# sangminwoo/Temporal-Span-Proposal-Network-VidVRD

Measured on AMD Instinct MI355X. Metric: tracklet-pairs/sec scored (N=32, T=150, D=2048), higher is better.
Workload: dtype f32

## Files before the change

temporal-span-proposal-network-vidvrd_amd/csrc/tspn_linear.hip:

```cpp
#include <algorithm>

#include "tspn_common.h"
#include "tspn_span_pool.h"
#include "tspn_device.h"

namespace {

using namespace tspn_dev;

constexpr int TM = 64;
constexpr int NBLK = 9;
constexpr int TN = 16 * NBLK;
constexpr int KC = 32;
constexpr int LDS_STRIDE = KC + 2;
constexpr int THREADS = 256;
constexpr int MAX_SPLIT = 64;

constexpr int MAX_NORM_SPLITS = 128;
struct SplitTable {
  int n;
  int kbeg[MAX_NORM_SPLITS];
  int kend[MAX_NORM_SPLITS];
  short blk[MAX_NORM_SPLITS];
};

template <bool NORM>
__global__ __launch_bounds__(THREADS) void linear_splitk_kernel(
    const float* __restrict__ x, int64_t P, int64_t F, int64_t ldx, const float* __restrict__ W,
    int64_t ldw, int64_t K, int64_t k_per_split, float* __restrict__ partial, SplitTable tab,
    float* __restrict__ norm_partial) {
  __shared__ float xs[TM * LDS_STRIDE];
  __shared__ float wsm[TN * LDS_STRIDE];

  const int tid = threadIdx.x;
  const int lane = tid & 63, wave = tid >> 6;
  const int li = lane & 15, kq = lane >> 4;
  const int64_t row0 = (int64_t)blockIdx.x * TM;
  const int64_t col0 = (int64_t)blockIdx.y * TN;
  int64_t kbeg, kend;
  if (NORM) {
    kbeg = tab.kbeg[blockIdx.z];
    kend = tab.kend[blockIdx.z];
  } else {
    kbeg = (int64_t)blockIdx.z * k_per_split;
    kend = (kbeg + k_per_split < F) ? kbeg + k_per_split : F;
  }
  float asum[TM / 8];
#pragma unroll
  for (int r = 0; r < TM / 8; ++r) asum[r] = 0.f;

  f32x4 acc[NBLK];
#pragma unroll
  for (int nb = 0; nb < NBLK; ++nb)
#pragma unroll
    for (int e = 0; e < 4; ++e) acc[nb][e] = 0.f;

  const int lk = tid & 31;
  const int lr = tid >> 5;

  for (int64_t k0 = kbeg; k0 < kend; k0 += KC) {
    const int64_t k = k0 + lk;
    const bool kv = k < kend;
#pragma unroll
    for (int r = 0; r < TM / 8; ++r) {
      const int row = lr + 8 * r;
      const int64_t gr = row0 + row;
      const float xv = (kv && gr < P) ? x[gr * ldx + k] : 0.f;
      xs[row * LDS_STRIDE + lk] = xv;
      if (NORM) asum[r] += fabsf(xv);
    }
#pragma unroll
    for (int r = 0; r < TN / 8; ++r) {
      const int row = lr + 8 * r;
      const int64_t gc = col0 + row;
      wsm[row * LDS_STRIDE + lk] = (kv && gc < K) ? W[gc * ldw + k] : 0.f;
    }
    __syncthreads();
#pragma unroll
    for (int kk = 0; kk < KC / 4; ++kk) {
      const float av = xs[(wave * 16 + li) * LDS_STRIDE + kk * 4 + kq];
#pragma unroll
      for (int nb = 0; nb < NBLK; ++nb) {
        const float bv = wsm[(nb * 16 + li) * LDS_STRIDE + kk * 4 + kq];
        acc[nb] = __builtin_amdgcn_mfma_f32_16x16x4f32(av, bv, acc[nb], 0, 0, 0);
      }
    }
    __syncthreads();
  }

  if (NORM && blockIdx.y == 0) {
#pragma unroll
    for (int r = 0; r < TM / 8; ++r) {
      float a = asum[r];
#pragma unroll
      for (int off = 16; off > 0; off >>= 1) a += __shfl_xor(a, off);
      const int64_t gr = row0 + lr + 8 * r;
      if (lk == 0 && gr < P) norm_partial[(int64_t)blockIdx.z * P + gr] = a;
    }
  }
  float* dst = partial + (int64_t)blockIdx.z * P * K;
#pragma unroll
  for (int nb = 0; nb < NBLK; ++nb) {
    const int64_t gc = col0 + nb * 16 + li;
    if (gc >= K) continue;
#pragma unroll
    for (int e = 0; e < 4; ++e) {
      const int64_t gr = row0 + wave * 16 + kq * 4 + e;
      if (gr < P) dst[gr * K + gc] = acc[nb][e];
    }
  }
}

__global__ void linear_reduce_kernel(const float* __restrict__ partial, int64_t PK, int64_t K,
                                     int splits, const float* __restrict__ b, int apply_sigmoid,
                                     float* __restrict__ out) {
  for (int64_t i = blockIdx.x * (int64_t)blockDim.x + threadIdx.x; i < PK;
       i += (int64_t)gridDim.x * blockDim.x) {
    float s = 0.f;
    for (int z = 0; z < splits; ++z) s += partial[(int64_t)z * PK + i];
    if (b != nullptr) s += b[i % K];
    if (apply_sigmoid) s = 1.f / (1.f + expf(-s));
    out[i] = s;
  }
}

__global__ void linear_reduce_norm_kernel(const float* __restrict__ partial,
                                          const float* __restrict__ norm_partial, int64_t P,
                                          int64_t K, SplitTable tab, const float* __restrict__ b,
                                          int apply_sigmoid, float* __restrict__ out) {
  const int64_t PK = P * K;
  for (int64_t i = blockIdx.x * (int64_t)blockDim.x + threadIdx.x; i < PK;
       i += (int64_t)gridDim.x * blockDim.x) {
    const int64_t row = i / K;
    float s = 0.f;
    int z = 0;
    while (z < tab.n) {
      const int blk = tab.blk[z];
      float acc = 0.f, l1 = 0.f;
      int z2 = z;
      for (; z2 < tab.n && tab.blk[z2] == blk; ++z2) {
        acc += partial[(int64_t)z2 * PK + i];
        if (blk >= 0) l1 += norm_partial[(int64_t)z2 * P + row];
      }
      if (blk >= 0) acc = acc / (l1 == 0.f ? 1.f : l1);
      s += acc;
      z = z2;
    }
    if (b != nullptr) s += b[i % K];
    if (apply_sigmoid) s = 1.f / (1.f + expf(-s));
    out[i] = s;
  }
}

int build_split_table(int64_t P, int64_t F, int64_t K, int64_t first, int64_t block, int64_t nblocks,
                      SplitTable* tab) {
  const int64_t tiles = tspn::ceil_div(P, TM) * tspn::ceil_div(K, TN);
  int64_t target = std::min<int64_t>(std::max<int64_t>(tspn::ceil_div(512, tiles), 1), 64);
  const int64_t len = std::max<int64_t>(tspn::ceil_div(tspn::ceil_div(F, target), KC) * KC, 2 * KC);
  int n = 0;
  auto add_region = [&](int64_t lo, int64_t hi, int blk) {
    if (hi <= lo) return true;
    const int64_t pieces = tspn::ceil_div(hi - lo, len);
    const int64_t step = tspn::ceil_div(tspn::ceil_div(hi - lo, pieces), KC) * KC;
    for (int64_t k = lo; k < hi; k += step) {
      if (n >= MAX_NORM_SPLITS) return false;
      tab->kbeg[n] = (int)k;
      tab->kend[n] = (int)std::min<int64_t>(k + step, hi);
      tab->blk[n] = (short)blk;
      ++n;
    }
    return true;
  };
  bool ok = add_region(0, first, -1);
  for (int64_t bl = 0; ok && bl < nblocks; ++bl)
    ok = add_region(first + bl * block, first + (bl + 1) * block, (int)bl);
  ok = ok && add_region(first + nblocks * block, F, -1);
  tab->n = n;
  return ok ? n : -1;
}

__global__ void pair_combine_kernel(const float* __restrict__ rs, const float* __restrict__ ro,
                                    const int64_t* __restrict__ pairs, int64_t P, int64_t K,
                                    const float* __restrict__ b, float* __restrict__ out) {
  const int64_t total = P * K;
  for (int64_t i = blockIdx.x * (int64_t)blockDim.x + threadIdx.x; i < total;
       i += (int64_t)gridDim.x * blockDim.x) {
    const int64_t p = i / K, k = i - p * K;
    float v = rs[pairs[2 * p] * K + k] + ro[pairs[2 * p + 1] * K + k];
    if (b != nullptr) v += b[k];
    out[i] = 1.f / (1.f + expf(-v));
  }
}

__global__ void span_prefix_kernel(const float* __restrict__ G, int64_t NT, int T, int K2,
                                   double* __restrict__ PS) {
  const int64_t total = NT * K2;
  for (int64_t i = blockIdx.x * (int64_t)blockDim.x + threadIdx.x; i < total;
       i += (int64_t)gridDim.x * blockDim.x) {
    const int64_t trk = i / K2, c = i - trk * K2;
    const float* g = G + (trk * T) * (int64_t)K2 + c;
    double* ps = PS + (trk * (T + 1)) * (int64_t)K2 + c;
    double acc = 0.0;
    ps[0] = 0.0;
    for (int t = 0; t < T; ++t) {
      acc += (double)g[(int64_t)t * K2];
      ps[(int64_t)(t + 1) * K2] = acc;
    }
  }
}

__global__ void span_combine_kernel(const double* __restrict__ PS, const float* __restrict__ G,
                                    const int64_t* __restrict__ pairs, const int64_t* __restrict__ spans,
                                    int64_t P, int T, int K, const float* __restrict__ b,
                                    float* __restrict__ out) {
  const int64_t total = P * K;
  const int64_t K2 = 2 * (int64_t)K;
  for (int64_t i = blockIdx.x * (int64_t)blockDim.x + threadIdx.x; i < total;
       i += (int64_t)gridDim.x * blockDim.x) {
    const int64_t p = i / K, k = i - p * K;
    out[i] = tspn::span_logit(PS, G, pairs[2 * p], pairs[2 * p + 1], spans[2 * p], spans[2 * p + 1], T, K2, k, b);
  }
}

int choose_splits(int64_t P, int64_t F, int64_t K) {
  const int64_t tiles = tspn::ceil_div(P, TM) * tspn::ceil_div(K, TN);
  int64_t s = tspn::ceil_div(512, tiles);
  s = std::min<int64_t>(s, std::max<int64_t>(1, F / (2 * KC)));
  s = std::min<int64_t>(s, MAX_SPLIT);
  return (int)std::max<int64_t>(s, 1);
}

}

extern "C" size_t tspn_predicate_head_workspace_bytes(int64_t P, int64_t F, int64_t K) {
  if (P <= 0 || F <= 0 || K <= 0) return 0;
  return (size_t)choose_splits(P, F, K) * (size_t)P * (size_t)K * sizeof(float);
}

extern "C" int tspn_predicate_head_f32(const float* x, int64_t P, int64_t F, int64_t ldx,
                                       const float* W, const float* b, int64_t K, float* out,
                                       int apply_sigmoid, void* workspace, size_t workspace_bytes,
                                       void* stream) {
  return tspn::linear(x, P, F, ldx, W, F, b, K, out, apply_sigmoid, workspace, workspace_bytes, stream);
}

int tspn::linear(const float* x, int64_t P, int64_t F, int64_t ldx, const float* W, int64_t ldw,
                 const float* b, int64_t K, float* out, int apply_sigmoid, void* workspace,
                 size_t workspace_bytes, void* stream) {
  TSPN_REQUIRE(ldw >= F, TSPN_EINVAL, "tspn_predicate_head_f32: bad ldw");
  TSPN_REQUIRE(P >= 0 && F > 0 && K > 0 && ldx >= F, TSPN_EINVAL,
               "tspn_predicate_head_f32: bad sizes P=%lld F=%lld K=%lld ldx=%lld", (long long)P,
               (long long)F, (long long)K, (long long)ldx);
  if (P == 0) return TSPN_OK;
  TSPN_REQUIRE(x && W && out, TSPN_EINVAL, "tspn_predicate_head_f32: null pointer");
  const int splits = choose_splits(P, F, K);
  const size_t need = (size_t)splits * (size_t)P * (size_t)K * sizeof(float);
  TSPN_REQUIRE(workspace != nullptr && workspace_bytes >= need, TSPN_EWORKSPACE,
               "tspn_predicate_head_f32: workspace %zu < %zu bytes", workspace_bytes, need);
  int64_t kps = tspn::ceil_div(F, splits);
  kps = tspn::ceil_div(kps, KC) * KC;
  const int64_t gx = tspn::ceil_div(P, TM), gy = tspn::ceil_div(K, TN);
  TSPN_REQUIRE(gx < (1LL << 31) && gy < 65536, TSPN_EUNSUPPORTED,
               "tspn_predicate_head_f32: grid too large");
  hipStream_t s = TSPN_STREAM(stream);
  float* partial = static_cast<float*>(workspace);
  hipLaunchKernelGGL(linear_splitk_kernel<false>, dim3((unsigned)gx, (unsigned)gy, (unsigned)splits),
                     dim3(THREADS), 0, s, x, P, F, ldx, W, ldw, K, kps, partial, SplitTable{},
                     (float*)nullptr);
  int rc = tspn::check_launch("tspn_predicate_head_f32(splitk)");
  if (rc) return rc;
  const int64_t PK = P * K;
  const int blocks = (int)std::min<int64_t>(tspn::ceil_div(PK, 256), 4096);
  hipLaunchKernelGGL(linear_reduce_kernel, dim3(blocks), dim3(256), 0, s, partial, PK, K, splits,
                     b, apply_sigmoid, out);
  return tspn::check_launch("tspn_predicate_head_f32(reduce)");
}

extern "C" size_t tspn_predicate_head_norm_workspace_bytes(int64_t P, int64_t F, int64_t K,
                                                           int64_t first, int64_t block,
                                                           int64_t nblocks) {
  if (P <= 0 || F <= 0 || K <= 0 || first < 0 || block <= 0 || nblocks < 0 ||
      first + block * nblocks > F)
    return 0;
  SplitTable tab;
  const int n = build_split_table(P, F, K, first, block, nblocks, &tab);
  if (n < 0) return 0;
  return (size_t)n * (size_t)P * (size_t)(K + 1) * sizeof(float);
}

extern "C" int tspn_predicate_head_norm_f32(const float* x, int64_t P, int64_t F, int64_t ldx,
                                            const float* W, const float* b, int64_t K,
                                            int64_t first, int64_t block, int64_t nblocks,
                                            float* out, int apply_sigmoid, void* workspace,
                                            size_t workspace_bytes, void* stream) {
  TSPN_REQUIRE(P >= 0 && F > 0 && K > 0 && ldx >= F, TSPN_EINVAL,
               "tspn_predicate_head_norm_f32: bad sizes P=%lld F=%lld K=%lld ldx=%lld", (long long)P,
               (long long)F, (long long)K, (long long)ldx);
  TSPN_REQUIRE(first >= 0 && block > 0 && nblocks >= 0 && first + block * nblocks <= F, TSPN_EINVAL,
               "tspn_predicate_head_norm_f32: blocks [%lld, %lld) exceed F=%lld", (long long)first,
               (long long)(first + block * nblocks), (long long)F);
  TSPN_REQUIRE(F < (1LL << 31) && nblocks < 32768, TSPN_EUNSUPPORTED,
               "tspn_predicate_head_norm_f32: F or nblocks too large");
  if (P == 0) return TSPN_OK;
  TSPN_REQUIRE(x && W && out, TSPN_EINVAL, "tspn_predicate_head_norm_f32: null pointer");
  SplitTable tab;
  const int n = build_split_table(P, F, K, first, block, nblocks, &tab);
  TSPN_REQUIRE(n > 0, TSPN_EUNSUPPORTED, "tspn_predicate_head_norm_f32: more than %d K-slices needed",
               MAX_NORM_SPLITS);
  const size_t need = (size_t)n * (size_t)P * (size_t)(K + 1) * sizeof(float);
  TSPN_REQUIRE(workspace != nullptr && workspace_bytes >= need, TSPN_EWORKSPACE,
               "tspn_predicate_head_norm_f32: workspace %zu < %zu bytes", workspace_bytes, need);
  const int64_t gx = tspn::ceil_div(P, TM), gy = tspn::ceil_div(K, TN);
  TSPN_REQUIRE(gx < (1LL << 31) && gy < 65536, TSPN_EUNSUPPORTED,
               "tspn_predicate_head_norm_f32: grid too large");
  hipStream_t s = TSPN_STREAM(stream);
  float* partial = static_cast<float*>(workspace);
  float* norm_partial = partial + (size_t)n * P * K;
  hipLaunchKernelGGL(linear_splitk_kernel<true>, dim3((unsigned)gx, (unsigned)gy, (unsigned)n),
                     dim3(THREADS), 0, s, x, P, F, ldx, W, F, K, (int64_t)0, partial, tab, norm_partial);
  int rc = tspn::check_launch("tspn_predicate_head_norm_f32(splitk)");
  if (rc) return rc;
  const int blocks = (int)std::min<int64_t>(tspn::ceil_div(P * K, 256), 4096);
  hipLaunchKernelGGL(linear_reduce_norm_kernel, dim3(blocks), dim3(256), 0, s, partial, norm_partial,
                     P, K, tab, b, apply_sigmoid, out);
  return tspn::check_launch("tspn_predicate_head_norm_f32(reduce)");
}

size_t tspn::pair_predicate_workspace_bytes(int64_t NT, int64_t D, int64_t K) {
  return tspn::align_up(tspn_predicate_head_workspace_bytes(NT, D, K), 256) +
         2 * tspn::align_up((size_t)NT * K * sizeof(float), 256);
}

int tspn::pair_predicate(const float* fbar, int64_t NT, int64_t D, const int64_t* pairs, int64_t P,
                         const float* cls_w, const float* cls_b, int64_t K, float* out,
                         void* workspace, size_t workspace_bytes, void* stream) {
  if (P == 0 || NT == 0) return TSPN_OK;
  const size_t lin = tspn::align_up(tspn_predicate_head_workspace_bytes(NT, D, K), 256);
  const size_t rbytes = tspn::align_up((size_t)NT * K * sizeof(float), 256);
  TSPN_REQUIRE(workspace && workspace_bytes >= lin + 2 * rbytes, TSPN_EWORKSPACE,
               "pair_predicate: workspace too small");
  char* ws = static_cast<char*>(workspace);
  float* rs = reinterpret_cast<float*>(ws + lin);
  float* ro = reinterpret_cast<float*>(ws + lin + rbytes);
  int rc = tspn::linear(fbar, NT, D, D, cls_w, 2 * D, nullptr, K, rs, 0, ws, lin, stream);
  if (rc) return rc;
  rc = tspn::linear(fbar, NT, D, D, cls_w + D, 2 * D, nullptr, K, ro, 0, ws, lin, stream);
  if (rc) return rc;
  const int blocks = (int)std::min<int64_t>(tspn::ceil_div(P * K, 256), 4096);
  hipLaunchKernelGGL(pair_combine_kernel, dim3(blocks), dim3(256), 0, TSPN_STREAM(stream), rs, ro, pairs,
                     P, K, cls_b, out);
  return tspn::check_launch("pair_predicate(combine)");
}

namespace {
struct SpanLayout {
  size_t lin, g, ps, total;
};
SpanLayout span_layout(int64_t NT, int64_t T, int64_t D, int64_t K) {
  SpanLayout L{};
  L.lin = tspn::align_up(tspn_predicate_head_workspace_bytes(NT * T, D, 2 * K), 256);
  L.g = tspn::align_up((size_t)NT * T * 2 * K * sizeof(float), 256);
  L.ps = tspn::align_up((size_t)NT * (T + 1) * 2 * K * sizeof(double), 256);
  L.total = L.lin + L.g + L.ps;
  return L;
}
}

size_t tspn::span_prefix_workspace_bytes(int64_t NT, int64_t T, int64_t D, int64_t K) {
  if (NT <= 0 || T <= 0 || D <= 0 || K <= 0) return 0;
  return span_layout(NT, T, D, K).total;
}

int tspn::span_prefix_stage(const float* feats, int64_t NT, int64_t T, int64_t D, const float* cls_w, int64_t K,
                            void* workspace, size_t workspace_bytes, void* stream, const float** G_out,
                            const double** PS_out, const char* who) {
  const SpanLayout L = span_layout(NT, T, D, K);
  TSPN_REQUIRE(workspace && workspace_bytes >= L.total, TSPN_EWORKSPACE, "%s: workspace %zu < %zu bytes", who,
               workspace_bytes, L.total);
  char* ws = static_cast<char*>(workspace);
  float* G = reinterpret_cast<float*>(ws + L.lin);
  double* PS = reinterpret_cast<double*>(ws + L.lin + L.g);
  int rc = tspn::linear(feats, NT * T, D, D, cls_w, D, nullptr, 2 * K, G, 0, ws, L.lin, stream);
  if (rc) return rc;
  const int b1 = (int)std::min<int64_t>(tspn::ceil_div(NT * 2 * K, 256), 8192);
  hipLaunchKernelGGL(span_prefix_kernel, dim3(b1), dim3(256), 0, TSPN_STREAM(stream), G, NT, (int)T, (int)(2 * K), PS);
  if ((rc = tspn::check_launch("tspn_span_predicate_f32(prefix)"))) return rc;
  *G_out = G;
  *PS_out = PS;
  return TSPN_OK;
}

extern "C" size_t tspn_span_predicate_workspace_bytes(int64_t NT, int64_t T, int64_t D, int64_t K) {
  return tspn::span_prefix_workspace_bytes(NT, T, D, K);
}

extern "C" int tspn_span_predicate_f32(const float* feats, int64_t NT, int64_t T, int64_t D,
                                       const int64_t* pairs, const int64_t* spans, int64_t P,
                                       const float* cls_w, const float* cls_b, int64_t K, float* out,
                                       void* workspace, size_t workspace_bytes, void* stream) {
  TSPN_REQUIRE(NT >= 0 && T > 0 && D > 0 && K > 0 && P >= 0 && T < (1 << 30) && K < (1 << 20), TSPN_EINVAL,
               "tspn_span_predicate_f32: bad sizes NT=%lld T=%lld D=%lld K=%lld P=%lld", (long long)NT,
               (long long)T, (long long)D, (long long)K, (long long)P);
  if (P == 0 || NT == 0) return TSPN_OK;
  TSPN_REQUIRE(feats && pairs && spans && cls_w && out, TSPN_EINVAL, "tspn_span_predicate_f32: null pointer");
  const float* G = nullptr;
  const double* PS = nullptr;
  int rc = tspn::span_prefix_stage(feats, NT, T, D, cls_w, K, workspace, workspace_bytes, stream, &G, &PS,
                                   "tspn_span_predicate_f32");
  if (rc) return rc;
  hipStream_t s = TSPN_STREAM(stream);
  const int b2 = (int)std::min<int64_t>(tspn::ceil_div(P * K, 256), 8192);
  hipLaunchKernelGGL(span_combine_kernel, dim3(b2), dim3(256), 0, s, PS, G, pairs, spans, P, (int)T,
                     (int)K, cls_b, out);
  return tspn::check_launch("tspn_span_predicate_f32(combine)");
}
```

temporal-span-proposal-network-vidvrd_amd/csrc/tspn_topk_select.h:

```cpp
#pragma once
#include "tspn_common.h"

namespace tspn {

constexpr unsigned kPadKey = 0u;
constexpr int kPadIdx = 0x7fffffff;

template <int THREADS>
__device__ __forceinline__ void bitonic_sort_desc(unsigned* key, int* idx, int n2) {
  const int tid = threadIdx.x;
  for (int k = 2; k <= n2; k <<= 1) {
    for (int j = k >> 1; j > 0; j >>= 1) {
      for (int i = tid; i < n2; i += THREADS) {
        const int l = i ^ j;
        if (l > i) {
          const unsigned ki = key[i], kl = key[l];
          const int ii = idx[i], il = idx[l];
          const bool fwd = (i & k) == 0;
          const bool swap = fwd ? key_before(kl, il, ki, ii) : key_before(ki, ii, kl, il);
          if (swap) {
            key[i] = kl;
            key[l] = ki;
            idx[i] = il;
            idx[l] = ii;
          }
        }
      }
      __syncthreads();
    }
  }
}

constexpr int kRowTopkVPT = 4;
constexpr int kRowTopkMaxK = 64 * kRowTopkVPT;

template <class Emit>
__device__ __forceinline__ void wave_row_topk(const float (&v)[kRowTopkVPT], int K, int R, int lane, Emit emit) {
  unsigned kv[kRowTopkVPT];
#pragma unroll
  for (int i = 0; i < kRowTopkVPT; ++i) kv[i] = order_key(v[i]);
  unsigned used = 0;
  for (int r = 0; r < R; ++r) {
    unsigned bk = kPadKey;
    int bi = kPadIdx;
#pragma unroll
    for (int i = 0; i < kRowTopkVPT; ++i) {
      const int k = lane + 64 * i;
      if (k < K && !((used >> i) & 1u) && key_before(kv[i], k, bk, bi)) {
        bk = kv[i];
        bi = k;
      }
    }
#pragma unroll
    for (int off = 32; off > 0; off >>= 1) {
      const unsigned ok = __shfl_xor(bk, off);
      const int oi = __shfl_xor(bi, off);
      if (key_before(ok, oi, bk, bi)) {
        bk = ok;
        bi = oi;
      }
    }
    if ((bi & 63) == lane && bi < K) {
      float bv = v[0];
#pragma unroll
      for (int i = 1; i < kRowTopkVPT; ++i)
        if ((bi >> 6) == i) bv = v[i];
      used |= 1u << (bi >> 6);
      emit(r, bv, bi);
    }
  }
}

constexpr int kSelectThreads = 1024;
constexpr int kSelectMaxM = 1024;

struct SelectLds {
  unsigned hist[256];
  unsigned prefix, need, count;
  unsigned kk[kSelectMaxM];
  int ki[kSelectMaxM];
};

template <class KeyFn>
__device__ __forceinline__ void select_topk_sorted(SelectLds& L, KeyFn key, int Q, int M) {
  const int tid = threadIdx.x;
  if (tid == 0) {
    L.prefix = 0;
    L.need = (unsigned)M;
  }
  __syncthreads();
  for (int pass = 0; pass < 4; ++pass) {
    const int shift = 24 - 8 * pass;
    if (tid < 256) L.hist[tid] = 0;
    __syncthreads();
    const unsigned prefix = L.prefix;
    const unsigned himask = pass == 0 ? 0u : (0xffffffffu << (shift + 8));
    for (int i = tid; i < Q; i += kSelectThreads) {
      const unsigned k = key(i);
      if ((k & himask) == prefix) atomicAdd(&L.hist[(k >> shift) & 255u], 1u);
    }
    __syncthreads();
    if (tid == 0) {
      unsigned need = L.need, acc = 0;
      int b = 255;
      for (; b >= 0; --b) {
        if (acc + L.hist[b] >= need) break;
        acc += L.hist[b];
      }
      L.prefix = prefix | ((unsigned)b << shift);
      L.need = need - acc;
    }
    __syncthreads();
  }
  const unsigned kth = L.prefix;
  const unsigned ties_needed = L.need;
  __syncthreads();
  if (tid == 0) {
    L.prefix = 0;
    L.need = ties_needed;
  }
  __syncthreads();
  for (int pass = 0; pass < 4; ++pass) {
    const int shift = 24 - 8 * pass;
    if (tid < 256) L.hist[tid] = 0;
    __syncthreads();
    const unsigned prefix = L.prefix;
    const unsigned himask = pass == 0 ? 0u : (0xffffffffu << (shift + 8));
    for (int i = tid; i < Q; i += kSelectThreads) {
      if (key(i) == kth && (((unsigned)i) & himask) == prefix)
        atomicAdd(&L.hist[(((unsigned)i) >> shift) & 255u], 1u);
    }
    __syncthreads();
    if (tid == 0) {
      unsigned need = L.need, acc = 0;
      int b = 0;
      for (; b < 256; ++b) {
        if (acc + L.hist[b] >= need) break;
        acc += L.hist[b];
      }
      L.prefix = prefix | ((unsigned)b << shift);
      L.need = need - acc;
    }
    __syncthreads();
  }
  const unsigned last_tie_idx = L.prefix;

  if (tid == 0) L.count = 0;
  __syncthreads();
  for (int i = tid; i < Q; i += kSelectThreads) {
    const unsigned k = key(i);
    if (k > kth || (k == kth && (unsigned)i <= last_tie_idx)) {
      const unsigned slot = atomicAdd(&L.count, 1u);
      if (slot < (unsigned)kSelectMaxM) {
        L.kk[slot] = k;
        L.ki[slot] = i;
      }
    }
  }
  __syncthreads();
  const int m2 = (int)next_pow2(M);
  for (int i = tid; i < m2; i += kSelectThreads)
    if (i >= M) {
      L.kk[i] = kPadKey;
      L.ki[i] = kPadIdx;
    }
  __syncthreads();
  bitonic_sort_desc<kSelectThreads>(L.kk, L.ki, m2);
}

__device__ inline int argmax_first(const float* p, int n) {
  unsigned bk = order_key(p[0]);
  int bi = 0;
  for (int i = 1; i < n; ++i) {
    const unsigned k = order_key(p[i]);
    if (k > bk) {
      bk = k;
      bi = i;
    }
  }
  return bi;
}

}
```

Baseline: 1.287 million.

## Batch pair-predicate GEMM halves and parallelize top-k selection primitives

```diff
diff --git a/temporal-span-proposal-network-vidvrd_amd/csrc/tspn_linear.hip b/temporal-span-proposal-network-vidvrd_amd/csrc/tspn_linear.hip
--- a/temporal-span-proposal-network-vidvrd_amd/csrc/tspn_linear.hip
+++ b/temporal-span-proposal-network-vidvrd_amd/csrc/tspn_linear.hip
@@ -28,7 +28,7 @@
 __global__ __launch_bounds__(THREADS) void linear_splitk_kernel(
     const float* __restrict__ x, int64_t P, int64_t F, int64_t ldx, const float* __restrict__ W,
     int64_t ldw, int64_t K, int64_t k_per_split, float* __restrict__ partial, SplitTable tab,
-    float* __restrict__ norm_partial) {
+    float* __restrict__ norm_partial, int gy, int64_t w_half, int64_t partial_half) {
   __shared__ float xs[TM * LDS_STRIDE];
   __shared__ float wsm[TN * LDS_STRIDE];
 
@@ -36,7 +36,9 @@
   const int lane = tid & 63, wave = tid >> 6;
   const int li = lane & 15, kq = lane >> 4;
   const int64_t row0 = (int64_t)blockIdx.x * TM;
-  const int64_t col0 = (int64_t)blockIdx.y * TN;
+  const int half = (int)blockIdx.y / gy;
+  const int64_t col0 = (int64_t)((int)blockIdx.y - half * gy) * TN;
+  W += half * w_half;
   int64_t kbeg, kend;
   if (NORM) {
     kbeg = tab.kbeg[blockIdx.z];
@@ -98,7 +100,7 @@
       if (lk == 0 && gr < P) norm_partial[(int64_t)blockIdx.z * P + gr] = a;
     }
   }
-  float* dst = partial + (int64_t)blockIdx.z * P * K;
+  float* dst = partial + half * partial_half + (int64_t)blockIdx.z * P * K;
 #pragma unroll
   for (int nb = 0; nb < NBLK; ++nb) {
     const int64_t gc = col0 + nb * 16 + li;
@@ -113,14 +115,16 @@
 
 __global__ void linear_reduce_kernel(const float* __restrict__ partial, int64_t PK, int64_t K,
                                      int splits, const float* __restrict__ b, int apply_sigmoid,
-                                     float* __restrict__ out) {
-  for (int64_t i = blockIdx.x * (int64_t)blockDim.x + threadIdx.x; i < PK;
-       i += (int64_t)gridDim.x * blockDim.x) {
+                                     float* __restrict__ out, int halves, int64_t partial_half, int64_t out_half) {
+  for (int64_t j = blockIdx.x * (int64_t)blockDim.x + threadIdx.x; j < halves * PK;
+       j += (int64_t)gridDim.x * blockDim.x) {
+    const int64_t half = j / PK, i = j - half * PK;
+    const float* src = partial + half * partial_half;
     float s = 0.f;
-    for (int z = 0; z < splits; ++z) s += partial[(int64_t)z * PK + i];
+    for (int z = 0; z < splits; ++z) s += src[(int64_t)z * PK + i];
     if (b != nullptr) s += b[i % K];
     if (apply_sigmoid) s = 1.f / (1.f + expf(-s));
-    out[i] = s;
+    out[half * out_half + i] = s;
   }
 }
 
@@ -244,9 +248,10 @@
   return tspn::linear(x, P, F, ldx, W, F, b, K, out, apply_sigmoid, workspace, workspace_bytes, stream);
 }
 
-int tspn::linear(const float* x, int64_t P, int64_t F, int64_t ldx, const float* W, int64_t ldw,
-                 const float* b, int64_t K, float* out, int apply_sigmoid, void* workspace,
-                 size_t workspace_bytes, void* stream) {
+namespace {
+int linear_halves(const float* x, int64_t P, int64_t F, int64_t ldx, const float* W, int64_t ldw, const float* b,
+                  int64_t K, float* out, int apply_sigmoid, void* workspace, size_t workspace_bytes, void* stream,
+                  int halves, int64_t w_half, int64_t out_half) {
   TSPN_REQUIRE(ldw >= F, TSPN_EINVAL, "tspn_predicate_head_f32: bad ldw");
   TSPN_REQUIRE(P >= 0 && F > 0 && K > 0 && ldx >= F, TSPN_EINVAL,
                "tspn_predicate_head_f32: bad sizes P=%lld F=%lld K=%lld ldx=%lld", (long long)P,
@@ -254,26 +259,34 @@
   if (P == 0) return TSPN_OK;
   TSPN_REQUIRE(x && W && out, TSPN_EINVAL, "tspn_predicate_head_f32: null pointer");
   const int splits = choose_splits(P, F, K);
-  const size_t need = (size_t)splits * (size_t)P * (size_t)K * sizeof(float);
+  const int64_t partial_half = (int64_t)splits * P * K;
+  const size_t need = (size_t)halves * (size_t)partial_half * sizeof(float);
   TSPN_REQUIRE(workspace != nullptr && workspace_bytes >= need, TSPN_EWORKSPACE,
                "tspn_predicate_head_f32: workspace %zu < %zu bytes", workspace_bytes, need);
   int64_t kps = tspn::ceil_div(F, splits);
   kps = tspn::ceil_div(kps, KC) * KC;
   const int64_t gx = tspn::ceil_div(P, TM), gy = tspn::ceil_div(K, TN);
-  TSPN_REQUIRE(gx < (1LL << 31) && gy < 65536, TSPN_EUNSUPPORTED,
+  TSPN_REQUIRE(gx < (1LL << 31) && halves * gy < 65536, TSPN_EUNSUPPORTED,
                "tspn_predicate_head_f32: grid too large");
   hipStream_t s = TSPN_STREAM(stream);
   float* partial = static_cast<float*>(workspace);
-  hipLaunchKernelGGL(linear_splitk_kernel<false>, dim3((unsigned)gx, (unsigned)gy, (unsigned)splits),
+  hipLaunchKernelGGL(linear_splitk_kernel<false>, dim3((unsigned)gx, (unsigned)(halves * gy), (unsigned)splits),
                      dim3(THREADS), 0, s, x, P, F, ldx, W, ldw, K, kps, partial, SplitTable{},
-                     (float*)nullptr);
+                     (float*)nullptr, (int)gy, w_half, partial_half);
   int rc = tspn::check_launch("tspn_predicate_head_f32(splitk)");
   if (rc) return rc;
   const int64_t PK = P * K;
-  const int blocks = (int)std::min<int64_t>(tspn::ceil_div(PK, 256), 4096);
+  const int blocks = (int)std::min<int64_t>(tspn::ceil_div(halves * PK, 256), 4096);
   hipLaunchKernelGGL(linear_reduce_kernel, dim3(blocks), dim3(256), 0, s, partial, PK, K, splits,
-                     b, apply_sigmoid, out);
+                     b, apply_sigmoid, out, halves, partial_half, out_half);
   return tspn::check_launch("tspn_predicate_head_f32(reduce)");
+}
+}
+
+int tspn::linear(const float* x, int64_t P, int64_t F, int64_t ldx, const float* W, int64_t ldw,
+                 const float* b, int64_t K, float* out, int apply_sigmoid, void* workspace,
+                 size_t workspace_bytes, void* stream) {
+  return linear_halves(x, P, F, ldx, W, ldw, b, K, out, apply_sigmoid, workspace, workspace_bytes, stream, 1, 0, 0);
 }
 
 extern "C" size_t tspn_predicate_head_norm_workspace_bytes(int64_t P, int64_t F, int64_t K,
@@ -317,7 +330,8 @@
   float* partial = static_cast<float*>(workspace);
   float* norm_partial = partial + (size_t)n * P * K;
   hipLaunchKernelGGL(linear_splitk_kernel<true>, dim3((unsigned)gx, (unsigned)gy, (unsigned)n),
-                     dim3(THREADS), 0, s, x, P, F, ldx, W, F, K, (int64_t)0, partial, tab, norm_partial);
+                     dim3(THREADS), 0, s, x, P, F, ldx, W, F, K, (int64_t)0, partial, tab, norm_partial, (int)gy,
+                     (int64_t)0, (int64_t)0);
   int rc = tspn::check_launch("tspn_predicate_head_norm_f32(splitk)");
   if (rc) return rc;
   const int blocks = (int)std::min<int64_t>(tspn::ceil_div(P * K, 256), 4096);
@@ -327,7 +341,7 @@
 }
 
 size_t tspn::pair_predicate_workspace_bytes(int64_t NT, int64_t D, int64_t K) {
-  return tspn::align_up(tspn_predicate_head_workspace_bytes(NT, D, K), 256) +
+  return tspn::align_up(2 * tspn_predicate_head_workspace_bytes(NT, D, K), 256) +
          2 * tspn::align_up((size_t)NT * K * sizeof(float), 256);
 }
 
@@ -335,20 +349,18 @@
                          const float* cls_w, const float* cls_b, int64_t K, float* out,
                          void* workspace, size_t workspace_bytes, void* stream) {
   if (P == 0 || NT == 0) return TSPN_OK;
-  const size_t lin = tspn::align_up(tspn_predicate_head_workspace_bytes(NT, D, K), 256);
+  const size_t lin = tspn::align_up(2 * tspn_predicate_head_workspace_bytes(NT, D, K), 256);
   const size_t rbytes = tspn::align_up((size_t)NT * K * sizeof(float), 256);
   TSPN_REQUIRE(workspace && workspace_bytes >= lin + 2 * rbytes, TSPN_EWORKSPACE,
                "pair_predicate: workspace too small");
   char* ws = static_cast<char*>(workspace);
   float* rs = reinterpret_cast<float*>(ws + lin);
-  float* ro = reinterpret_cast<float*>(ws + lin + rbytes);
-  int rc = tspn::linear(fbar, NT, D, D, cls_w, 2 * D, nullptr, K, rs, 0, ws, lin, stream);
-  if (rc) return rc;
-  rc = tspn::linear(fbar, NT, D, D, cls_w + D, 2 * D, nullptr, K, ro, 0, ws, lin, stream);
+  int rc = linear_halves(fbar, NT, D, D, cls_w, 2 * D, nullptr, K, rs, 0, ws, lin, stream, 2, D,
+                         (int64_t)(rbytes / sizeof(float)));
   if (rc) return rc;
   const int blocks = (int)std::min<int64_t>(tspn::ceil_div(P * K, 256), 4096);
-  hipLaunchKernelGGL(pair_combine_kernel, dim3(blocks), dim3(256), 0, TSPN_STREAM(stream), rs, ro, pairs,
-                     P, K, cls_b, out);
+  hipLaunchKernelGGL(pair_combine_kernel, dim3(blocks), dim3(256), 0, TSPN_STREAM(stream), rs,
+                     rs + rbytes / sizeof(float), pairs, P, K, cls_b, out);
   return tspn::check_launch("pair_predicate(combine)");
 }
 
diff --git a/temporal-span-proposal-network-vidvrd_amd/csrc/tspn_topk_select.h b/temporal-span-proposal-network-vidvrd_amd/csrc/tspn_topk_select.h
--- a/temporal-span-proposal-network-vidvrd_amd/csrc/tspn_topk_select.h
+++ b/temporal-span-proposal-network-vidvrd_amd/csrc/tspn_topk_select.h
@@ -36,43 +36,67 @@
 
 template <class Emit>
 __device__ __forceinline__ void wave_row_topk(const float (&v)[kRowTopkVPT], int K, int R, int lane, Emit emit) {
-  unsigned kv[kRowTopkVPT];
-#pragma unroll
-  for (int i = 0; i < kRowTopkVPT; ++i) kv[i] = order_key(v[i]);
-  unsigned used = 0;
-  for (int r = 0; r < R; ++r) {
-    unsigned bk = kPadKey;
-    int bi = kPadIdx;
-#pragma unroll
-    for (int i = 0; i < kRowTopkVPT; ++i) {
-      const int k = lane + 64 * i;
-      if (k < K && !((used >> i) & 1u) && key_before(kv[i], k, bk, bi)) {
-        bk = kv[i];
-        bi = k;
+  static_assert(kRowTopkVPT == 4, "the sort network below is written for 4 slots per lane");
+  unsigned sk[kRowTopkVPT];
+  int si[kRowTopkVPT];
+#pragma unroll
+  for (int i = 0; i < kRowTopkVPT; ++i) {
+    const int k = lane + 64 * i;
+    sk[i] = k < K ? order_key(v[i]) : kPadKey;
+    si[i] = k;
+  }
+#pragma unroll
+  for (int kk = 2; kk <= kRowTopkMaxK; kk <<= 1) {
+#pragma unroll
+    for (int j = kk >> 1; j > 0; j >>= 1) {
+      if (j >= kRowTopkVPT) {
+        const int lj = j / kRowTopkVPT;
+        const bool keep_best = ((lane & lj) == 0) == (((kRowTopkVPT * lane) & kk) == 0);
+#pragma unroll
+        for (int s = 0; s < kRowTopkVPT; ++s) {
+          const unsigned ok = __shfl_xor(sk[s], lj);
+          const int oi = __shfl_xor(si[s], lj);
+          if (key_before(ok, oi, sk[s], si[s]) == keep_best) {
+            sk[s] = ok;
+            si[s] = oi;
+          }
+        }
+      } else {
+#pragma unroll
+        for (int a = 0; a < kRowTopkVPT; ++a) {
+          const int b = a | j;
+          if (b == a) continue;
+          const bool desc = ((kRowTopkVPT * lane + a) & kk) == 0;
+          if (key_before(sk[b], si[b], sk[a], si[a]) == desc) {
+            const unsigned tk = sk[a];
+            const int ti = si[a];
+            sk[a] = sk[b];
+            si[a] = si[b];
+            sk[b] = tk;
+            si[b] = ti;
+          }
+        }
       }
     }
-#pragma unroll
-    for (int off = 32; off > 0; off >>= 1) {
-      const unsigned ok = __shfl_xor(bk, off);
-      const int oi = __shfl_xor(bi, off);
-      if (key_before(ok, oi, bk, bi)) {
-        bk = ok;
-        bi = oi;
+  }
+  for (int r0 = 0; r0 < R; r0 += kRowTopkVPT) {
+#pragma unroll
+    for (int s = 0; s < kRowTopkVPT; ++s) {
+      const int k = __builtin_amdgcn_readlane(si[s], r0 / kRowTopkVPT);
+      if (r0 + s < R && (k & 63) == lane) {
+        unsigned bv = 0;
+#pragma unroll
+        for (int i = 0; i < kRowTopkVPT; ++i) bv |= __float_as_uint(v[i]) & (0u - (unsigned)((k >> 6) == i));
+        emit(r0 + s, __uint_as_float(bv), k);
       }
-    }
-    if ((bi & 63) == lane && bi < K) {
-      float bv = v[0];
-#pragma unroll
-      for (int i = 1; i < kRowTopkVPT; ++i)
-        if ((bi >> 6) == i) bv = v[i];
-      used |= 1u << (bi >> 6);
-      emit(r, bv, bi);
     }
   }
 }
 
 constexpr int kSelectThreads = 1024;
 constexpr int kSelectMaxM = 1024;
+constexpr int kSelectRegKeys = 32;
+constexpr int kSelectRegCap = kSelectRegKeys * kSelectThreads;
 
 struct SelectLds {
   unsigned hist[256];
@@ -81,9 +105,88 @@
   int ki[kSelectMaxM];
 };
 
+template <class KeyFn, class F>
+__device__ __forceinline__ void select_for_each(const unsigned (&regs)[kSelectRegKeys], bool in_regs, KeyFn key, int Q,
+                                                F f) {
+  const int tid = threadIdx.x;
+  if (in_regs) {
+#pragma unroll
+    for (int j = 0; j < kSelectRegKeys; ++j) {
+      if (j * kSelectThreads >= Q) break;
+      const int i = tid + j * kSelectThreads;
+      f(regs[j], i, i < Q);
+    }
+  } else {
+    for (int base = 0; base < Q; base += kSelectThreads) {
+      const int i = base + tid;
+      f(i < Q ? key(i) : kPadKey, i, i < Q);
+    }
+  }
+}
+
+__device__ __forceinline__ void select_hist_add(unsigned* hist, bool on, unsigned b) {
+  const int lane = threadIdx.x & 63;
+  unsigned long long rem = __ballot(on);
+#pragma unroll
+  for (int round = 0; round < 2; ++round) {
+    if (rem == 0) break;
+    const int lead = __ffsll((long long)rem) - 1;
+    const unsigned b0 = (unsigned)__builtin_amdgcn_readlane((int)b, lead);
+    const unsigned long long same = __ballot(on && b == b0);
+    if (lane == lead) atomicAdd(&hist[b0], (unsigned)__popcll(same));
+    on = on && b != b0;
+    rem &= ~same;
+  }
+  if (on) atomicAdd(&hist[b], 1u);
+}
+
+template <bool DESC>
+__device__ __forceinline__ void select_find_bucket(SelectLds& L, unsigned prefix, int shift) {
+  const int lane = threadIdx.x & 63;
+  const unsigned need = L.need;
+  unsigned c[4], sum = 0;
+#pragma unroll
+  for (int j = 0; j < 4; ++j) {
+    const int o = 4 * lane + j, b = DESC ? 255 - o : o;
+    c[j] = L.hist[b];
+    L.hist[b] = 0;
+    sum += c[j];
+  }
+  unsigned inc = sum;
+#pragma unroll
+  for (int off = 1; off < 64; off <<= 1) {
+    const unsigned t = __shfl_up(inc, off);
+    if (lane >= off) inc += t;
+  }
+  const unsigned long long hit = __ballot(inc >= need);
+  const int first = hit ? __ffsll((long long)hit) - 1 : 63;
+  if (lane == first) {
+    unsigned acc = inc - sum;
+    int j = 0;
+    for (; j < 3; ++j) {
+      if (acc + c[j] >= need) break;
+      acc += c[j];
+    }
+    const int o = 4 * lane + j, b = DESC ? 255 - o : o;
+    L.prefix = prefix | ((unsigned)b << shift);
+    L.need = need - acc;
+    L.count = c[j];
+  }
+}
+
 template <class KeyFn>
 __device__ __forceinline__ void select_topk_sorted(SelectLds& L, KeyFn key, int Q, int M) {
   const int tid = threadIdx.x;
+  const bool in_regs = Q <= kSelectRegCap;
+  unsigned regs[kSelectRegKeys];
+  if (in_regs) {
+#pragma unroll
+    for (int j = 0; j < kSelectRegKeys; ++j) {
+      const int i = tid + j * kSelectThreads;
+      regs[j] = i < Q ? key(i) : kPadKey;
+    }
+  }
+  if (tid < 256) L.hist[tid] = 0;
   if (tid == 0) {
     L.prefix = 0;
     L.need = (unsigned)M;
@@ -91,72 +194,58 @@
   __syncthreads();
   for (int pass = 0; pass < 4; ++pass) {
     const int shift = 24 - 8 * pass;
-    if (tid < 256) L.hist[tid] = 0;
-    __syncthreads();
     const unsigned prefix = L.prefix;
     const unsigned himask = pass == 0 ? 0u : (0xffffffffu << (shift + 8));
-    for (int i = tid; i < Q; i += kSelectThreads) {
-      const unsigned k = key(i);
-      if ((k & himask) == prefix) atomicAdd(&L.hist[(k >> shift) & 255u], 1u);
-    }
-    __syncthreads();
-    if (tid == 0) {
-      unsigned need = L.need, acc = 0;
-      int b = 255;
-      for (; b >= 0; --b) {
-        if (acc + L.hist[b] >= need) break;
-        acc += L.hist[b];
-      }
-      L.prefix = prefix | ((unsigned)b << shift);
-      L.need = need - acc;
-    }
+    select_for_each(regs, in_regs, key, Q, [&](unsigned k, int, bool valid) {
+      select_hist_add(L.hist, valid && (k & himask) == prefix, (k >> shift) & 255u);
+    });
+    __syncthreads();
+    if (tid < 64) select_find_bucket<true>(L, prefix, shift);
     __syncthreads();
   }
   const unsigned kth = L.prefix;
   const unsigned ties_needed = L.need;
-  __syncthreads();
-  if (tid == 0) {
-    L.prefix = 0;
-    L.need = ties_needed;
-  }
-  __syncthreads();
-  for (int pass = 0; pass < 4; ++pass) {
-    const int shift = 24 - 8 * pass;
-    if (tid < 256) L.hist[tid] = 0;
-    __syncthreads();
-    const unsigned prefix = L.prefix;
-    const unsigned himask = pass == 0 ? 0u : (0xffffffffu << (shift + 8));
-    for (int i = tid; i < Q; i += kSelectThreads) {
-      if (key(i) == kth && (((unsigned)i) & himask) == prefix)
-        atomicAdd(&L.hist[(((unsigned)i) >> shift) & 255u], 1u);
-    }
-    __syncthreads();
+  const unsigned ties = L.count;
+  __syncthreads();
+  unsigned last_tie_idx = 0xffffffffu;
+  if (ties_needed < ties) {
     if (tid == 0) {
-      unsigned need = L.need, acc = 0;
-      int b = 0;
-      for (; b < 256; ++b) {
-        if (acc + L.hist[b] >= need) break;
-        acc += L.hist[b];
-      }
-      L.prefix = prefix | ((unsigned)b << shift);
-      L.need = need - acc;
-    }
-    __syncthreads();
-  }
-  const unsigned last_tie_idx = L.prefix;
+      L.prefix = 0;
+      L.need = ties_needed;
+    }
+    __syncthreads();
+    for (int pass = 0; pass < 4; ++pass) {
+      const int shift = 24 - 8 * pass;
+      const unsigned prefix = L.prefix;
+      const unsigned himask = pass == 0 ? 0u : (0xffffffffu << (shift + 8));
+      select_for_each(regs, in_regs, key, Q, [&](unsigned k, int i, bool valid) {
+        select_hist_add(L.hist, valid && k == kth && (((unsigned)i) & himask) == prefix, (((unsigned)i) >> shift) & 255u);
+      });
+      __syncthreads();
+      if (tid < 64) select_find_bucket<false>(L, prefix, shift);
+      __syncthreads();
+    }
+    last_tie_idx = L.prefix;
+    __syncthreads();
+  }
 
   if (tid == 0) L.count = 0;
   __syncthreads();
-  for (int i = tid; i < Q; i += kSelectThreads) {
-    const unsigned k = key(i);
-    if (k > kth || (k == kth && (unsigned)i <= last_tie_idx)) {
-      const unsigned slot = atomicAdd(&L.count, 1u);
-      if (slot < (unsigned)kSelectMaxM) {
-        L.kk[slot] = k;
-        L.ki[slot] = i;
-      }
-    }
-  }
+  const int lane = tid & 63;
+  select_for_each(regs, in_regs, key, Q, [&](unsigned k, int i, bool valid) {
+    const bool win = valid && (k > kth || (k == kth && (unsigned)i <= last_tie_idx));
+    const unsigned long long won = __ballot(win);
+    if (won == 0) return;
+    const int lead = __ffsll((long long)won) - 1;
+    unsigned base = 0;
+    if (lane == lead) base = atomicAdd(&L.count, (unsigned)__popcll(won));
+    base = (unsigned)__builtin_amdgcn_readlane((int)base, lead);
+    const unsigned slot = base + __builtin_amdgcn_mbcnt_hi((unsigned)(won >> 32), __builtin_amdgcn_mbcnt_lo((unsigned)won, 0u));
+    if (win && slot < (unsigned)kSelectMaxM) {
+      L.kk[slot] = k;
+      L.ki[slot] = i;
+    }
+  });
   __syncthreads();
   const int m2 = (int)next_pow2(M);
   for (int i = tid; i < m2; i += kSelectThreads)
```

Result: no change. 1.295 million (median of 6 runs) (+0.6%).
